# Leonhard111/M3L

Measured on AMD Instinct MI355X. Metric: MAE fwd+bwd samples/sec (image+tactile), higher is better.
Workload: dtype bf16; 1 GPU; BASELINE configs[1]: VTT vision+tactile MAE, 64x64 RGB + 2x32x32 tactile, ViT-Tiny 192/12/3/768 + decoder 192/4/3/768, mask 0.75; batch_per_gpu=256, global_batch=256, parallelism=dp1, grad_allreduce=none (one rank), rccl_ranks=0, step=zero_grad + mask + fwd + bwd + grad all-reduce + Adam

## Files before the change

include/m3l_amd.h:

```cpp
#ifndef M3L_AMD_H
#define M3L_AMD_H
#include <stddef.h>
#include <stdint.h>

#ifdef __cplusplus
extern "C" {
#endif

#define M3L_MAX_TACTILES 8

typedef struct m3l_geom {
    int image_h, image_w, image_patch, image_channels;
    int tactile_h, tactile_w, tactile_patch, tactile_channels;
    int num_tactiles;
    int use_vision;
    int use_tactile;
} m3l_geom;

typedef struct m3l_tf_cfg {
    int dim, depth, heads, mlp_dim;
    int project_out;
    int dtype;
    int dim_head;
} m3l_tf_cfg;

typedef struct m3l_dropout {
    float p;
    uint64_t seed;
} m3l_dropout;

int m3l_version(void);
int m3l_last_error(char* buf, size_t n);
int m3l_set_rowln(int enable);
int m3l_set_attn_block(int mode);
int m3l_set_enc_mega(int mode);
void m3l_set_attn_phase_buffer(void* dev_buf);
int m3l_set_defer_join(int on);
int m3l_set_wgrad_inline(int on);
int m3l_side_join(void* stream);
int m3l_comm_available(void);
int m3l_comm_unique_id(void* out128);
int m3l_comm_init(const void* id128, int rank, int world);
int m3l_comm_world(void);
int m3l_comm_allreduce(float* buf, size_t count, void* after_stream);
int m3l_comm_destroy(void);
int m3l_side_fork(void* after_stream, void** side_out);
int m3l_side_mark_pending(void);
void* m3l_side_stream(void);
int m3l_side_pending(void);
int m3l_set_drop_h(int on);
int m3l_set_t192(int on);
int m3l_set_t192_tt(int tt);
int m3l_set_residual_bf16(int on);
int m3l_set_t192_stagger(int lead_mask, int prio_mask);

int m3l_mask_counts(const m3l_geom* g, double ratio, int* counts_host);
int m3l_mask_sample(const m3l_geom* g, double ratio, int B, const float* const* noise, int64_t* masked, int64_t* unmasked,
                    void* stream);

int m3l_mask_sample_counts(const m3l_geom* g, int nm_img, int nm_tac, int B, const float* const* noise, int64_t* masked,
                           int64_t* unmasked, void* stream);

size_t m3l_embed_ws_bytes(const m3l_geom* g, int D, int dtype, int B, int L);
int m3l_embed_fwd(const m3l_geom* g, int D, int dtype, int B, int L, int cnt_img, const int64_t* idx, const float* image,
                  const float* const* tactiles, const void* const* tensors, void* ws, float* tokens, void* stream);
int m3l_embed_bwd(const m3l_geom* g, int D, int dtype, int B, int L, int cnt_img, const int64_t* idx, const float* image,
                  const float* const* tactiles, const void* const* tensors, void* ws, const float* dtokens, float* const* grads,
                  void* stream);

size_t m3l_transformer_ws_bytes(const m3l_tf_cfg* c, int B, int n);
int m3l_transformer_fwd(const m3l_tf_cfg* c, int B, int n, const float* x_in, const void* const* tensors, void* ws, void* y_t,
                        float* y32, void* stream);
int m3l_transformer_bwd(const m3l_tf_cfg* c, int B, int n, const float* x_in, const void* const* tensors, void* ws, const void* dy,
                        int dy_dtype, float* dx_in, float* const* grads, void* stream);

int m3l_transformer_bwd_range(const m3l_tf_cfg* c, int B, int n, const float* x_in, const void* const* tensors, void* ws,
                              const void* dy, int dy_dtype, float* dx_in, float* const* grads, int layer_hi, int layer_lo, void* stream);

size_t m3l_transformer_ws_bytes_dropout(const m3l_tf_cfg* c, int B, int n, const m3l_dropout* drop);
int m3l_transformer_fwd_dropout(const m3l_tf_cfg* c, int B, int n, const float* x_in, const void* const* tensors, void* ws, void* y_t,
                                float* y32, const m3l_dropout* drop, void* stream);
int m3l_transformer_bwd_dropout(const m3l_tf_cfg* c, int B, int n, const float* x_in, const void* const* tensors, void* ws, const void* dy,
                                int dy_dtype, float* dx_in, float* const* grads, const m3l_dropout* drop, void* stream);
int m3l_transformer_bwd_range_dropout(const m3l_tf_cfg* c, int B, int n, const float* x_in, const void* const* tensors, void* ws,
                                      const void* dy, int dy_dtype, float* dx_in, float* const* grads, int layer_hi, int layer_lo,
                                      const m3l_dropout* drop, void* stream);

// ... 163 lines not shown
```

m3l_amd/_lib.py:

```python
import ctypes as C
import os

_HERE = os.path.dirname(os.path.abspath(__file__))
LIB_PATH = os.environ.get("M3L_LIB_PATH") or os.path.join(_HERE, "lib", "libm3l_amd.so")

c_p = C.c_void_p
c_i = C.c_int
c_sz = C.c_size_t


class Geom(C.Structure):
    _fields_ = [(n, c_i) for n in ("image_h", "image_w", "image_patch", "image_channels", "tactile_h", "tactile_w",
                                   "tactile_patch", "tactile_channels", "num_tactiles", "use_vision", "use_tactile")]


class CnnCfg(C.Structure):
    _fields_ = [(n, c_i) for n in ("in_channels", "height", "width", "dim", "tactile", "dtype")]


class TfCfg(C.Structure):
    _fields_ = [(n, c_i) for n in ("dim", "depth", "heads", "mlp_dim", "project_out", "dtype", "dim_head")]


class MaeCfg(C.Structure):
    _fields_ = [("geom", Geom), ("enc", TfCfg), ("dec", TfCfg), ("masking_ratio", C.c_double), ("early_conv", c_i), ("learned_pos", c_i)]


class Dropout(C.Structure):
    _fields_ = [("p", C.c_float), ("seed", C.c_uint64)]


class CommPlan(C.Structure):
    _fields_ = [("flat", c_p), ("total", C.c_long), ("min_bucket", C.c_long), ("layers_per_chunk", c_i), ("n_stages", c_i),
                ("stage_end", C.POINTER(C.c_long)), ("sent_out", C.POINTER(C.c_long))]


_SIGS = {
    "m3l_version": (c_i, []),
    "m3l_last_error": (c_i, [C.c_char_p, c_sz]),
    "m3l_set_rowln": (c_i, [c_i]),
    "m3l_set_attn_block": (c_i, [c_i]),
    "m3l_set_attn_phase_buffer": (None, [c_p]),
    "m3l_set_enc_mega": (c_i, [c_i]),
    "m3l_set_drop_h": (c_i, [c_i]),
    "m3l_set_direct_conv": (c_i, [c_i]),
    "m3l_set_t192": (c_i, [c_i]),
    "m3l_set_t192_tt": (c_i, [c_i]),
    "m3l_set_t192_stagger": (c_i, [c_i, c_i]),
    "m3l_set_residual_bf16": (c_i, [c_i]),
    "m3l_set_defer_join": (c_i, [c_i]),
    "m3l_set_wgrad_inline": (c_i, [c_i]),
    "m3l_side_join": (c_i, [c_p]),
    "m3l_side_stream": (c_p, []),
    "m3l_side_fork": (c_i, [c_p, C.POINTER(c_p)]),
    "m3l_side_mark_pending": (c_i, []),
    "m3l_comm_available": (c_i, []),
    "m3l_comm_unique_id": (c_i, [c_p]),
    "m3l_comm_init": (c_i, [c_p, c_i, c_i]),
    "m3l_comm_world": (c_i, []),
    "m3l_comm_allreduce": (c_i, [c_p, c_sz, c_p]),
    "m3l_comm_destroy": (c_i, []),
    "m3l_side_pending": (c_i, []),
    "m3l_mask_counts": (c_i, [C.POINTER(Geom), C.c_double, C.POINTER(c_i)]),
    "m3l_mask_sample": (c_i, [C.POINTER(Geom), C.c_double, c_i, c_p, c_p, c_p, c_p]),
    "m3l_mask_sample_counts": (c_i, [C.POINTER(Geom), c_i, c_i, c_i, c_p, c_p, c_p, c_p]),
    "m3l_embed_ws_bytes": (c_sz, [C.POINTER(Geom), c_i, c_i, c_i, c_i]),
    "m3l_embed_fwd": (c_i, [C.POINTER(Geom), c_i, c_i, c_i, c_i, c_i, c_p, c_p, c_p, c_p, c_p, c_p, c_p]),
    "m3l_embed_bwd": (c_i, [C.POINTER(Geom), c_i, c_i, c_i, c_i, c_i, c_p, c_p, c_p, c_p, c_p, c_p, c_p, c_p]),
    "m3l_transformer_ws_bytes": (c_sz, [C.POINTER(TfCfg), c_i, c_i]),
    "m3l_transformer_fwd": (c_i, [C.POINTER(TfCfg), c_i, c_i, c_p, c_p, c_p, c_p, c_p, c_p]),
    "m3l_transformer_bwd": (c_i, [C.POINTER(TfCfg), c_i, c_i, c_p, c_p, c_p, c_p, c_i, c_p, c_p, c_p]),
    "m3l_transformer_bwd_range": (c_i, [C.POINTER(TfCfg), c_i, c_i, c_p, c_p, c_p, c_p, c_i, c_p, c_p, c_i, c_i, c_p]),
    "m3l_transformer_ws_bytes_dropout": (c_sz, [C.POINTER(TfCfg), c_i, c_i, C.POINTER(Dropout)]),
    "m3l_transformer_fwd_dropout": (c_i, [C.POINTER(TfCfg), c_i, c_i, c_p, c_p, c_p, c_p, c_p, C.POINTER(Dropout), c_p]),
    "m3l_transformer_bwd_dropout": (c_i, [C.POINTER(TfCfg), c_i, c_i, c_p, c_p, c_p, c_p, c_i, c_p, c_p, C.POINTER(Dropout), c_p]),
    "m3l_transformer_bwd_range_dropout": (c_i, [C.POINTER(TfCfg), c_i, c_i, c_p, c_p, c_p, c_p, c_i, c_p, c_p, c_i, c_i, C.POINTER(Dropout), c_p]),
    "m3l_frozen_vit_ws_bytes": (c_sz, [C.POINTER(TfCfg), c_i, c_i]),
    "m3l_frozen_vit_fwd": (c_i, [C.POINTER(TfCfg), C.c_float, c_i, c_i, c_p, c_p, c_p, c_p, c_p]),
    "m3l_unshuffle_ws_bytes": (c_sz, [C.POINTER(Geom), c_i, c_i, c_i, c_i, c_i, c_i]),
    "m3l_unshuffle_fwd": (c_i, [C.POINTER(Geom), c_i, c_i, c_i, c_i, c_i, c_i, c_p, c_p, c_p, c_p, c_p, c_p, c_p, c_p]),
    "m3l_unshuffle_bwd": (c_i, [C.POINTER(Geom), c_i, c_i, c_i, c_i, c_i, c_i, c_p, c_p, c_p, c_p, c_p, c_p, c_p,
# ... 128 lines not shown
```

m3l_amd/csrc/t192.hip:

```cpp
#include <hip/hip_runtime.h>
#include <stdlib.h>
#include <string.h>

#include <algorithm>

#include "common.cuh"
#include "kernels.h"

namespace {


#ifndef T192_ABL
#define T192_ABL 0
#endif
#ifndef T192_NS_TALL
#define T192_NS_TALL 4
#endif
template <int D, int TT, int CP> struct TileCfg {
    static constexpr int KS = D / 32, ND = D / 16;
    static constexpr int BLK = 64 * D;
    static constexpr int CHUNK = 2 * BLK;
    static constexpr int PCB = D / 16, PC = 2 * PCB;
    static constexpr bool HALF = D == 192 && TT == 6 && CP == 1;
    static constexpr int DW = (D == 384 || HALF) ? 2 : 4;
// ... 23 lines not shown
    return v;
}
__device__ __forceinline__ float col4_sum(float v) {
    v = xor16_sum(v);
    v = xor32_sum(v);
    return v;
}

__device__ __forceinline__ int f1_swz(int row) { return ((row >> 1) & 1) | (((row >> 3) & 3) << 1); }
__device__ __forceinline__ Frag<bf16> frag_f1p(const char* blk, int t, int ks, int li, int g) {
    const int row = 8 * (li >> 2) + 4 * t + (li & 3);
    Frag<bf16> f;
    f.v = *reinterpret_cast<const bf16x8*>(blk + (ks >> 1) * 4096 + row * 128 + ((((ks & 1) * 4 + g) ^ f1_swz(row)) << 4));
    return f;
}
__device__ __forceinline__ int f2_swz(int row) { return (4 - (row >> 2)) & 3; }
__device__ __forceinline__ Frag<bf16> frag_f2(const char* blk, int dt, int li, int g) {
    const int row = 16 * dt + li;
    Frag<bf16> f;
    f.v = *reinterpret_cast<const bf16x8*>(blk + row * 64 + ((g ^ f2_swz(row)) << 4));
    return f;
}

__device__ __forceinline__ void dma_f1_piece(const bf16* W, int ldw, int r0, int p, char* dst, int lane) {
    const int kt = p >> 2, rg = p & 3;
    const int row = 8 * rg + (lane >> 3), csrc = (lane & 7) ^ f1_swz(row);
    __builtin_amdgcn_global_load_lds((gl_vp)(W + (long)(r0 + row) * ldw + kt * 64 + csrc * 8), (lds_vp)(dst + kt * 4096 + rg * 1024), 16, 0, 0);
}
__device__ __forceinline__ void dma_f2_piece(const bf16* W, int ldw, int c0, int p, char* dst, int lane) {
    const int row = 16 * p + (lane >> 2), csrc = (lane & 3) ^ f2_swz(row);
    __builtin_amdgcn_global_load_lds((gl_vp)(W + (long)row * ldw + c0 + csrc * 8), (lds_vp)(dst + p * 1024), 16, 0, 0);
}

template <int D, int TT, int CP, int LK = 0, typename Issue>
__device__ __forceinline__ void dma_ring(int dw, int nc, char* ring, Issue issue, int tail) {
    using Cf = TileCfg<D, TT, CP>;
    constexpr int LOOK = LK > 0 ? LK : Cf::NSTAGE - 1;
    const int nst = (nc + CP - 1) / CP;
    auto stage = [&](int s) {
        char* dst = ring + (s % Cf::NSTAGE) * Cf::STAGE;
#pragma unroll
        for (int j = 0; j < Cf::PPW; ++j) {
            const int p = dw * Cf::PPW + j, q = p / Cf::PC;
            issue(min(s * CP + q, nc - 1), dst + q * Cf::CHUNK, p % Cf::PC);
        }
    };
    for (int s = 0; s < LOOK && s < nst; ++s) stage(s);
    for (int s = 0; s < nst; ++s) {
        const int ahead = min(LOOK - 1, nst - 1 - s);
        if (ahead >= 4) wait_vmcnt<(LOOK >= 5 ? 4 : 0) * Cf::PPW>();
        else if (ahead == 3) wait_vmcnt<(LOOK >= 4 ? 3 : 0) * Cf::PPW>();
        else if (ahead == 2) wait_vmcnt<(LOOK >= 3 ? 2 : 0) * Cf::PPW>();
        else if (ahead == 1) wait_vmcnt<Cf::PPW>();
        else wait_vmcnt<0>();
        __builtin_amdgcn_s_barrier();
        if (s + LOOK < nst) stage(s + LOOK);
    }
    for (int i = 0; i < tail; ++i) __builtin_amdgcn_s_barrier();
}

template <int KS>
__device__ __forceinline__ void load_tok_frags(const bf16* __restrict__ X, long lrow, bool ok, int g, Frag<bf16> (&fb)[KS]) {
    constexpr int D = 32 * KS;
    uint4 v[KS];
#pragma unroll
    for (int ks = 0; ks < KS; ++ks) v[ks] = *reinterpret_cast<const uint4*>(X + lrow * D + ks * 32 + 8 * g);
#pragma unroll
    for (int ks = 0; ks < KS; ++ks) fb[ks].v = __builtin_bit_cast(bf16x8, ok ? v[ks] : uint4{0u, 0u, 0u, 0u});
}
__device__ __forceinline__ __amdgpu_buffer_rsrc_t rows_rsrc(const void* p, long bytes) {
    return __builtin_amdgcn_make_buffer_rsrc(const_cast<void*>(p), 0, p ? (int)bytes : 0, 0x00020000);
}
constexpr int ROW_OOB = 0x7fffffff;
__device__ __forceinline__ void store_row16(__amdgpu_buffer_rsrc_t r, int rowoff, int byteoff, f32x4 v) {
    __builtin_amdgcn_raw_buffer_store_b128(__builtin_bit_cast(u4v_t, v), r, (int)((unsigned)rowoff + (unsigned)byteoff), 0, 0);
}
__device__ __forceinline__ void store_row8(__amdgpu_buffer_rsrc_t r, int rowoff, int byteoff, bf16x4 v) {
    __builtin_amdgcn_raw_buffer_store_b64(__builtin_bit_cast(u2v_t, v), r, (int)((unsigned)rowoff + (unsigned)byteoff), 0, 0);
}

template <typename R> __device__ __forceinline__ void store_res4(__amdgpu_buffer_rsrc_t r, int rowoff, int col, f32x4 v) {
    if (sizeof(R) == 4) store_row16(r, rowoff, col * 4, v);
    else store_row8(r, rowoff, col * 2, pack_bf16x4(v));
}

template <int TT, int CP, int ND>
// ... 194 lines not shown
        }
#pragma unroll
        for (int st2 = KS; st2 < 2 * KS; ++st2) {
            const Frag<bf16> a0 = fr[st2 % PFD][0], a1 = fr[st2 % PFD][1];
            asm volatile("" ::: "memory");
            if (st2 + PFD < 2 * KS) req(st2 + PFD, fr[st2 % PFD]);
            asm volatile("" ::: "memory");
            if (!(T192_ABL & 4)) {
            yacc[2 * (st2 - KS)] = mma16(a0, hb, yacc[2 * (st2 - KS)]);
            yacc[2 * (st2 - KS) + 1] = mma16(a1, hb, yacc[2 * (st2 - KS) + 1]);
            } else { yacc[2 * (st2 - KS)][0] += (float)hb.v[st2 & 7]; }
        }
    }
    reduce_to_parity0<TT, CP, ND>(RING, tw, cp, lane, yacc);
    if (cp == 0 && (!(T192_ABL & 8) || yacc[0][0] == 1234.5f)) {
        f32x4 r1[ND];
#pragma unroll
        for (int d = 0; d < ND; ++d) r1[d] = ld_res4<R>(x1 + lrow * D + 16 * d + 4 * g);
        asm volatile("" ::: "memory");
        const __amdgpu_buffer_rsrc_t rxo = rows_rsrc(xout, (long)M * D * sizeof(R));
#pragma unroll
        for (int d = 0; d < ND; ++d) {
            const int col = 16 * d + 4 * g;
            const f32x4 v = yacc[d] + *reinterpret_cast<const f32x4*>(B2 + col) + r1[d];
            store_res4<R>(rxo, xoff, col, v);
        }
    }
}

template <int D, int TT, int CP> struct MlpBwdLayout {
    static constexpr bool CS_LDS = D == 192 && !TileCfg<D, TT, CP>::HALF && (CP > 1 || T192_NS_TALL <= 4);
    static constexpr int RING = 0, CS = TileCfg<D, TT, CP>::RING;
    static size_t total(int mlp) { return (size_t)CS + (CS_LDS ? (size_t)TT * mlp * 4 : 0) + D * 4; }
};

template <int ND, typename R>
__device__ __forceinline__ void ln_bwd_rows(const f32x4 (&yacc)[ND], const R* __restrict__ x, const float* G,
                                            const R* __restrict__ dres, R* __restrict__ dx_out, bf16* __restrict__ dxt_out, float eps,
                                            long trow, long lrow, long M, bool active, char* lp_base, int wave, int lane) {
    constexpr int T_D = 16 * ND;
    const int g = lane >> 4, li = lane & 15;
    constexpr int BT = ND % 6 == 0 ? 6 : 4;
    static_assert(ND % BT == 0, "ND is a multiple of the batch");
    const bool use = active && !(T192_ABL & 32);
    const R* xr = x + lrow * T_D + 4 * g;
    float s = 0.f;
#pragma unroll
    for (int d0 = 0; d0 < ND; d0 += BT) {
        f32x4 v[BT];
#pragma unroll
        for (int j = 0; j < BT; ++j) v[j] = ld_res4<R>(xr + 16 * (d0 + j));
#pragma unroll
        for (int j = 0; j < BT; ++j) {
            if (!use) v[j] = f32x4{0.f, 0.f, 0.f, (float)(d0 + j)};
            s += (v[j][0] + v[j][1]) + (v[j][2] + v[j][3]);
        }
    }
    const float mean = col4_sum(s) * (1.0f / T_D);
    asm volatile("" : "+v"(xr));
    float q = 0.f, s1 = 0.f, t2 = 0.f;
#pragma unroll
    for (int d0 = 0; d0 < ND; d0 += BT) {
        f32x4 v[BT];
#pragma unroll
        for (int j = 0; j < BT; ++j) v[j] = ld_res4<R>(xr + 16 * (d0 + j));
#pragma unroll
        for (int j = 0; j < BT; ++j) {
            const int d = d0 + j;
            if (!use) v[j] = f32x4{0.f, 0.f, 0.f, (float)d};
            const f32x4 xc = v[j] - mean;
            q += (xc[0] * xc[0] + xc[1] * xc[1]) + (xc[2] * xc[2] + xc[3] * xc[3]);
            const f32x4 gd = yacc[d] * *reinterpret_cast<const f32x4*>(G + 16 * d + 4 * g);
            s1 += (gd[0] + gd[1]) + (gd[2] + gd[3]);
            const f32x4 t = gd * xc;
            t2 += (t[0] + t[1]) + (t[2] + t[3]);
        }
    }
    const float rstd = rsqrtf(col4_sum(q) * (1.0f / T_D) + eps);
    s1 = col4_sum(s1) * (1.0f / T_D);
    const float s2 = col4_sum(t2) * rstd * (1.0f / T_D);
    asm volatile("" : "+v"(xr));
    __builtin_amdgcn_s_barrier();
    float* LP = reinterpret_cast<float*>(lp_base) + wave * 3 * T_D;
    const int roff32 = use ? (int)(trow * T_D * sizeof(R)) : ROW_OOB, roff16 = use ? (int)(trow * T_D * 2) : ROW_OOB;
    const __amdgpu_buffer_rsrc_t rdx = rows_rsrc(dx_out, M * T_D * sizeof(R)), rdt = rows_rsrc(dxt_out, M * T_D * 2);
    constexpr int BO = 4;
    static_assert(ND % BO == 0, "ND is a multiple of the batch");
    const R* dr_ = dres + lrow * T_D + 4 * g;
#pragma unroll
    for (int d0 = 0; d0 < ND; d0 += BO) {
        f32x4 v[BO], dr[BO];
#pragma unroll
        for (int j = 0; j < BO; ++j) {
            v[j] = ld_res4<R>(xr + 16 * (d0 + j));
            dr[j] = ld_res4<R>(dr_ + 16 * (d0 + j));
        }
        asm volatile("" ::: "memory");
#pragma unroll
        for (int j = 0; j < BO; ++j) {
            const int d = d0 + j, col = 16 * d + 4 * g;
            if (!use) v[j] = f32x4{0.f, 0.f, 0.f, (float)d};
            const f32x4 xh = (v[j] - mean) * rstd;
            const f32x4 gd = yacc[d] * *reinterpret_cast<const f32x4*>(G + col);
            f32x4 rr = f32x4{0.f, 0.f, 0.f, 0.f};
            if (active) rr = (gd - s1 - xh * s2) * rstd;
            if (use) rr += dr[j];
            store_res4<R>(rdx, roff32, col, rr);
            bf16x4 pk;
            pk[0] = (bf16)rr[0]; pk[1] = (bf16)rr[1]; pk[2] = (bf16)rr[2]; pk[3] = (bf16)rr[3];
            store_row8(rdt, roff16, col * 2, pk);
            f32x4 pg = yacc[d] * xh, pb = yacc[d], pc = rr;
            if (!active) { pg = f32x4{0.f, 0.f, 0.f, 0.f}; pb = pg; }
#pragma unroll
            for (int e = 0; e < 4; ++e) {
                pg[e] = row16_sum_t(pg[e]); pb[e] = row16_sum_t(pb[e]); pc[e] = row16_sum_t(pc[e]);
            }
            if (li == 0) {
                *reinterpret_cast<f32x4*>(LP + col) = pg;
                *reinterpret_cast<f32x4*>(LP + T_D + col) = pb;
                *reinterpret_cast<f32x4*>(LP + 2 * T_D + col) = pc;
            }
        }
    }
    asm volatile("s_waitcnt lgkmcnt(0)" ::: "memory");
    __builtin_amdgcn_s_barrier();
}

template <int D, int TT, int CP, typename R>
__global__ __launch_bounds__((TileCfg<D, TT, CP>::THREADS), (TileCfg<D, TT, CP>::MINW)) void mlp_t192_bwd_kernel(const bf16* __restrict__ dxt, R* __restrict__ dx,
                                                                   const R* __restrict__ x1, const float* __restrict__ ln2_w,
                                                                   const bf16* __restrict__ u, const bf16* __restrict__ W2T,
                                                                   const bf16* __restrict__ W1T, float eps, int M, int mlp,
                                                                   bf16* __restrict__ du_out, bf16* __restrict__ dx1t_out,
                                                                   float* __restrict__ cs_part, float* __restrict__ ln_part) {
    using Cf = TileCfg<D, TT, CP>;
    using Lay = MlpBwdLayout<D, TT, CP>;
    constexpr int NCW = Cf::NCW, KS = Cf::KS, ND = Cf::ND;
    static_assert(Lay::CS_LDS || CP == 1, "global column-sum rows are per (tile, wave)");
    extern __shared__ __attribute__((aligned(16))) char smem[];
    char* RING = smem + Lay::RING;
    float* CS = reinterpret_cast<float*>(smem + Lay::CS);
    float* G = Lay::CS_LDS ? CS + TT * mlp : CS;
    const int tid = threadIdx.x, lane = tid & 63, wave = __builtin_amdgcn_readfirstlane(tid >> 6);
    const int g = lane >> 4, li = lane & 15;
    const long row0 = (long)blockIdx.x * Cf::ROWS;
    const int NC = mlp >> 5;
    const int NS = (NC + CP - 1) / CP;

    if (wave >= NCW) {
        dma_ring<D, TT, CP>(wave - NCW, NC, RING, [&](int c, char* dst, int p) {
            if (p < Cf::PCB) dma_f1_piece(W2T, D, 32 * c, p, dst, lane);
            else dma_f2_piece(W1T, mlp, 32 * c, p - Cf::PCB, dst + Cf::BLK, lane);
        }, CP > 1 ? 5 : 3);
        return;
    }
    const int tw = wave % TT, cp = wave / TT;
    const long trow = row0 + 16 * tw + li;
    const bool ok = trow < M;
    Frag<bf16> db[KS];
    load_tok_frags(dxt, ok ? trow : (long)M - 1, ok, g, db);
    for (int id = tid; id < D; id += 64 * NCW) G[id] = ln2_w[id];
    float* CSw = Lay::CS_LDS ? CS + tw * mlp : cs_part + ((long)blockIdx.x * TT + tw) * mlp;

    f32x4 yacc[ND];
#pragma unroll
    for (int d = 0; d < ND; ++d) yacc[d] = f32x4{0.f, 0.f, 0.f, 0.f};
    uint4 un = uint4{0u, 0u, 0u, 0u};
    if (ok && cp < NC) un = *reinterpret_cast<const uint4*>(u + trow * mlp + 32 * cp + 8 * g);

    for (int st = 0; st < NS; ++st) {
        __builtin_amdgcn_s_barrier();
        asm volatile("" ::: "memory");
        const int c = st * CP + cp;
        if (c >= NC) continue;
        const Frag<bf16> uc = {__builtin_bit_cast(bf16x8, un)};
        if (ok && c + CP < NC && !(T192_ABL & 128)) un = *reinterpret_cast<const uint4*>(u + trow * mlp + 32 * (c + CP) + 8 * g);
        const char* Wa = RING + (st % Cf::NSTAGE) * Cf::STAGE + cp * Cf::CHUNK;
        const char* Wb = Wa + Cf::BLK;
        f32x4 ta[2] = {f32x4{0.f, 0.f, 0.f, 0.f}, f32x4{0.f, 0.f, 0.f, 0.f}};
        Frag<bf16> fr[PFD][2];
        auto req = [&](int step, Frag<bf16>(&dst)[2]) {
            if (step < KS) {
                dst[0] = frag_f1p(Wa, 0, step, li, g);
                dst[1] = frag_f1p(Wa, 1, step, li, g);
            } else {
                dst[0] = frag_f2(Wb, 2 * (step - KS), li, g);
                dst[1] = frag_f2(Wb, 2 * (step - KS) + 1, li, g);
            }
        };
#pragma unroll
        for (int i = 0; i < PFD; ++i) req(i, fr[i]);
#pragma unroll
        for (int ks = 0; ks < KS; ++ks) {
            const Frag<bf16> a0 = fr[ks % PFD][0], a1 = fr[ks % PFD][1];
            asm volatile("" ::: "memory");
            req(ks + PFD, fr[ks % PFD]);
            asm volatile("" ::: "memory");
            ta[0] = mma16(a0, db[ks], ta[0]);
            ta[1] = mma16(a1, db[ks], ta[1]);
        }
        Frag<bf16> dub;
#pragma unroll
        for (int j = 0; j < 8; ++j) {
            const float t = j < 4 ? ta[0][j & 3] : ta[1][j & 3];
            dub.v[j] = (bf16)(t * gelu_grad_fast((float)uc.v[j]));
        }
        if (ok && !(T192_ABL & 64)) *reinterpret_cast<bf16x8*>(du_out + trow * mlp + 32 * c + 8 * g) = dub.v;
        {
            float cs[8];
#pragma unroll
            for (int j = 0; j < 8; ++j) cs[j] = row16_sum_t(ok ? (float)dub.v[j] : 0.f);
            if (li == 0) {
                *reinterpret_cast<f32x4*>(CSw + 32 * c + 8 * g) = f32x4{cs[0], cs[1], cs[2], cs[3]};
                *reinterpret_cast<f32x4*>(CSw + 32 * c + 8 * g + 4) = f32x4{cs[4], cs[5], cs[6], cs[7]};
            }
        }
#pragma unroll
        for (int st2 = KS; st2 < 2 * KS; ++st2) {
            const Frag<bf16> a0 = fr[st2 % PFD][0], a1 = fr[st2 % PFD][1];
            asm volatile("" ::: "memory");
            if (st2 + PFD < 2 * KS) req(st2 + PFD, fr[st2 % PFD]);
            asm volatile("" ::: "memory");
            yacc[2 * (st2 - KS)] = mma16(a0, dub, yacc[2 * (st2 - KS)]);
            yacc[2 * (st2 - KS) + 1] = mma16(a1, dub, yacc[2 * (st2 - KS) + 1]);
        }
    }
    reduce_to_parity0<TT, CP, ND>(RING, tw, cp, lane, yacc);
    {
        const R* dres = dx;
        if (sizeof(R) == 2) dres = reinterpret_cast<const R*>(dxt);
        ln_bwd_rows<ND, R>(yacc, x1, G, dres, sizeof(R) == 2 ? nullptr : dx, dx1t_out, eps, trow, ok ? trow : (long)M - 1, M, ok && cp == 0, RING, wave, lane);
    }
    {
        const float* LP0 = reinterpret_cast<const float*>(RING);
        for (int id = tid; id < 3 * D; id += 64 * NCW) {
            float a = 0.f;
#pragma unroll
            for (int w = 0; w < TT; ++w) a += LP0[w * 3 * D + id];
            ln_part[(long)blockIdx.x * 3 * D + id] = a;
        }
        if (Lay::CS_LDS) {
            for (int id = tid; id < mlp; id += 64 * NCW) {
                float a = 0.f;
#pragma unroll
                for (int w = 0; w < TT; ++w) a += CS[w * mlp + id];
                cs_part[(long)blockIdx.x * mlp + id] = a;
            }
        }
    }
    __builtin_amdgcn_s_barrier();
}

template <int D, int TT, int CP>
__global__ __launch_bounds__((TileCfg<D, TT, CP>::THREADS), (TileCfg<D, TT, CP>::MINW)) void mlp_t192_bwd_stg_kernel(const bf16* __restrict__ dxt, float* __restrict__ dx,
                                                                   const float* __restrict__ x1, const float* __restrict__ ln2_w,
                                                                   const bf16* __restrict__ u, const bf16* __restrict__ W2T,
                                                                   const bf16* __restrict__ W1T, float eps, int M, int mlp,
                                                                   bf16* __restrict__ du_out, bf16* __restrict__ dx1t_out,
                                                                   float* __restrict__ cs_part, float* __restrict__ ln_part, int lead_mask, int prio_mask) {
    using Cf = TileCfg<D, TT, CP>;
// ... 694 lines not shown
    if (!(t192_state() > 0 && dtype == 1 && width_ok(D) && mlp % 32 == 0 && mlp >= 32 && M > 0 && rows_fit_32bit(D, M))) return 0;
    if (D == 192) return mlp <= 1024;
    return mlp <= 2048 && (M >= wide_min_rows(D) || forced());
}

static int t192_min_tiles() {
    static const int v = getenv("M3L_T192_MIN_TILES") ? atoi(getenv("M3L_T192_MIN_TILES")) : 128;
    return v;
}
static int g_tall_tt = 0;
static int tall_tt() {
    if (!g_tall_tt) g_tall_tt = (getenv("M3L_T192_TT") && atoi(getenv("M3L_T192_TT")) == 6) ? 6 : 12;
    return g_tall_tt;
}
extern "C" int m3l_set_t192_tt(int tt) {
    const int old = tall_tt();
    g_tall_tt = tt == 6 ? 6 : 12;
    return old;
}
static int g_stg = -1, g_prio = 0;
static void stg_init() {
    if (g_stg < 0) {
        g_stg = getenv("M3L_T192_STG") ? (int)strtol(getenv("M3L_T192_STG"), nullptr, 0) : 0;
        g_prio = getenv("M3L_T192_PRIO") ? (int)strtol(getenv("M3L_T192_PRIO"), nullptr, 0) : 0;
    }
}
extern "C" int m3l_set_t192_stagger(int lead_mask, int prio_mask) {
    stg_init();
    const int old = g_stg;
    g_stg = lead_mask & 0x1fff;
    g_prio = prio_mask & 0xfff;
    return old;
}
static int t192_tt(int M) { return (cdiv(M, 192) >= t192_min_tiles() || forced()) ? tall_tt() : 3; }
static int tile_rows(int D, int M) { return D == 192 ? 16 * t192_tt(M) : 16 * (D == 256 ? WideTile<256>::TT : WideTile<384>::TT); }
int m3l_mlp_t192_tiles(int D, int M) { return cdiv(M, tile_rows(D, M)); }
int m3l_mlp_t192_cs_rows(int D, int M) {
    const int tt = tile_rows(D, M) / 16;
    const bool cs_lds = D == 192 && tt != 6 && (tt == 3 || T192_NS_TALL <= 4);
    return m3l_mlp_t192_tiles(D, M) * (cs_lds ? 1 : tt);
}

template <typename K> static int lds_attr(K kern, size_t bytes) {
    M3L_HIP(hipFuncSetAttribute((const void*)kern, hipFuncAttributeMaxDynamicSharedMemorySize, (int)std::min(bytes, (size_t)160 * 1024)));
    return 0;
}
#define LDS_ONCE(KERN, BYTES)                               \
    {                                                       \
        static int once = -1;                               \
        if (once < 0) once = lds_attr(KERN, BYTES);         \
        if (once) return once;                              \
    }
#define T192_DISPATCH(DV, TTV, ...)                                                                    \
    if ((DV) == 192 && (TTV) == 12) { constexpr int D = 192, TT = 12, CP = 1; __VA_ARGS__; }           \
    else if ((DV) == 192 && (TTV) == 6) { constexpr int D = 192, TT = 6, CP = 1; __VA_ARGS__; }        \
    else if ((DV) == 192) { constexpr int D = 192, TT = 3, CP = 2; __VA_ARGS__; }                      \
    else if ((DV) == 256) { constexpr int D = 256, TT = WideTile<256>::TT, CP = 1; __VA_ARGS__; }      \
    else { constexpr int D = 384, TT = WideTile<384>::TT, CP = 1; __VA_ARGS__; }
#define T192_DISPATCH_FULL(DV, ...)                                                                    \
    if ((DV) == 192 && tall_tt() == 12) { constexpr int D = 192, TT = 12, CP = 1; __VA_ARGS__; }       \
    else if ((DV) == 192) { constexpr int D = 192, TT = 6, CP = 1; __VA_ARGS__; }                      \
    else if ((DV) == 256) { constexpr int D = 256, TT = WideTile<256>::TT, CP = 1; __VA_ARGS__; }      \
    else { constexpr int D = 384, TT = WideTile<384>::TT, CP = 1; __VA_ARGS__; }

#define T192_RES(...)                                            \
    if (m3l_call_rb()) { using R = bf16; __VA_ARGS__; }           \
// ... 27 lines not shown
    const int tt = Dm == 192 ? t192_tt(M) : tile_rows(Dm, M) / 16;
    const double rsz = m3l_call_rb() ? 2.0 : 4.0;
    ProfScope prof("mlp_t192_fwd", M, mlp, tt, 4.0 * M * (double)Dm * mlp, st, (double)M * (Dm * 2.0 + 2.0 * rsz * Dm + mlp * (h ? 4.0 : 2.0)));
    ProArgs none;
    memset(&none, 0, sizeof(none));
    T192_DISPATCH(Dm, tt, T192_RES({
        LDS_ONCE((mlp_t192_fwd_kernel<D, TT, CP, 0, R>), (MlpFwdLayout<D, TT, CP>::total(D == 192 ? 1024 : 2048)));
        mlp_t192_fwd_kernel<D, TT, CP, 0, R><<<cdiv(M, 16 * TT), TileCfg<D, TT, CP>::THREADS, MlpFwdLayout<D, TT, CP>::total(mlp), st>>>(
            (const bf16*)xn2, (const R*)x1, (const bf16*)w1, b1, (const bf16*)w2, b2, M, mlp, (bf16*)u, (bf16*)h, (R*)xout, none);
    }));
    M3L_LAUNCH_CHECK();
    return 0;
}

int m3l_attn_tail_mlp_t192_supported(int dtype, int D, int HD, int mlp, int M, int dim_head) {
    if (!(m3l_mlp_t192_supported(dtype, D, mlp, M) && HD == D && dim_head == 64)) return 0;
    return D != 192 || cdiv(M, 192) >= t192_min_tiles() || forced();
}
int m3l_attn_tail_mlp_t192_fwd(int Dm, int M, int mlp, const void* o, const float* x, const void* wo, const float* bo, const float* ln2_w,
                               const float* ln2_b, float eps, float* x1, void* xn2, const void* w1, const float* b1, const void* w2,
                               const float* b2, void* u, void* h, float* xout, hipStream_t st) {
    M3L_CHECK(width_ok(Dm), "attn_tail_mlp_t192_fwd: width %d", Dm);
    ProfScope prof("attn_tail_mlp_t192_fwd", M, mlp, Dm == 192 ? tall_tt() : tile_rows(Dm, M) / 16, 4.0 * M * (double)Dm * mlp + 2.0 * M * (double)Dm * Dm, st,
                   (double)M * (Dm * 4.0 + 3.0 * (m3l_call_rb() ? 2.0 : 4.0) * Dm + mlp * (h ? 4.0 : 2.0)));
    ProArgs pa = {(const bf16*)o, x, (const bf16*)wo, bo, ln2_w, ln2_b, eps, x1, (bf16*)xn2};
    T192_DISPATCH_FULL(Dm, T192_RES({
        LDS_ONCE((mlp_t192_fwd_kernel<D, TT, CP, 1, R>), (MlpFwdLayout<D, TT, CP>::total(D == 192 ? 1024 : 2048)));
        mlp_t192_fwd_kernel<D, TT, CP, 1, R><<<cdiv(M, 16 * TT), TileCfg<D, TT, CP>::THREADS, MlpFwdLayout<D, TT, CP>::total(mlp), st>>>(
            nullptr, nullptr, (const bf16*)w1, b1, (const bf16*)w2, b2, M, mlp, (bf16*)u, (bf16*)h, (R*)xout, pa);
    }));
    M3L_LAUNCH_CHECK();
    return 0;
}

int m3l_mlp_t192_bwd(int Dm, int M, int mlp, const void* dxt, float* dx, const float* x1, const float* ln2_w, const void* u, const void* w2T,
                     const void* w1T, float eps, void* du, void* dx1t, float* cs_part, float* ln_part, hipStream_t st) {
    M3L_CHECK(width_ok(Dm), "mlp_t192_bwd: width %d", Dm);
    const int tt = Dm == 192 ? t192_tt(M) : tile_rows(Dm, M) / 16;
    ProfScope prof("mlp_t192_bwd", M, mlp, tt, 4.0 * M * (double)Dm * mlp, st,
                   (double)M * (Dm * 4.0 + (m3l_call_rb() ? 2.0 : 12.0) * Dm + mlp * 4.0));
    T192_DISPATCH(Dm, tt, T192_RES({
        LDS_ONCE((mlp_t192_bwd_kernel<D, TT, CP, R>), (MlpBwdLayout<D, TT, CP>::total(D == 192 ? 1024 : 2048)));
        M3L_CHECK((MlpBwdLayout<D, TT, CP>::total(mlp)) <= (size_t)160 * 1024, "mlp_t192_bwd: %zu bytes of LDS", (MlpBwdLayout<D, TT, CP>::total(mlp)));
        stg_init();
        const int stg = g_stg, prio = g_prio;
        if constexpr (D == 192 && TT == 12 && CP == 1 && T192_NS_TALL == 4 && sizeof(R) == 4) {
            if (stg || prio) {
                LDS_ONCE((mlp_t192_bwd_stg_kernel<D, TT, CP>), (MlpBwdLayout<D, TT, CP>::total(1024)));
                mlp_t192_bwd_stg_kernel<D, TT, CP><<<cdiv(M, 16 * TT), TileCfg<D, TT, CP>::THREADS, MlpBwdLayout<D, TT, CP>::total(mlp), st>>>(
                    (const bf16*)dxt, dx, x1, ln2_w, (const bf16*)u, (const bf16*)w2T, (const bf16*)w1T, eps, M, mlp, (bf16*)du, (bf16*)dx1t, cs_part,
                    ln_part, stg & 0xfff, prio);
                M3L_LAUNCH_CHECK();
                return 0;
            }
        }
        mlp_t192_bwd_kernel<D, TT, CP, R><<<cdiv(M, 16 * TT), TileCfg<D, TT, CP>::THREADS, MlpBwdLayout<D, TT, CP>::total(mlp), st>>>(
            (const bf16*)dxt, (R*)dx, (const R*)x1, ln2_w, (const bf16*)u, (const bf16*)w2T, (const bf16*)w1T, eps, M, mlp, (bf16*)du, (bf16*)dx1t, cs_part,
            ln_part);
    }));
    M3L_LAUNCH_CHECK();
    return 0;
}

int m3l_qkv_bwd_t192_supported(int dtype, int D, int K, int M) {
    if (!(t192_state() > 0 && dtype == 1 && width_ok(D) && K % 64 == 0 && K >= 64 && M > 0 && rows_fit_32bit(D, M))) return 0;
    if (D == 192) return cdiv(M, 192) >= t192_min_tiles() || forced();
    return M >= wide_min_rows(D) || forced();
}
int m3l_qkv_bwd_t192_tiles(int D, int M) { return cdiv(M, D == 192 ? 16 * tall_tt() : tile_rows(D, M)); }

int m3l_qkv_bwd_t192(int Dm, int M, int K, const void* dqkv, const float* x, const float* ln1_w, const void* wqkvT, const float* dres, float eps,
                     float* dx_out, void* dxt_out, float* ln_part, hipStream_t st) {
    M3L_CHECK(width_ok(Dm), "qkv_bwd_t192: width %d", Dm);
    ProfScope prof("qkv_bwd_t192", M, K, Dm, 2.0 * M * (double)Dm * K, st,
                   (double)M * (K * 2.0 + Dm * 2.0 + (m3l_call_rb() ? 4.0 : 12.0) * Dm));
    T192_DISPATCH_FULL(Dm, T192_RES({
        LDS_ONCE((qkv_bwd_t192_kernel<D, TT, R>), (QkvBwdLayout<D, TT>::TOTAL));
        qkv_bwd_t192_kernel<D, TT, R><<<cdiv(M, 16 * TT), TileCfg<D, TT, CP>::THREADS, QkvBwdLayout<D, TT>::TOTAL, st>>>(
            (const bf16*)dqkv, (const R*)x, ln1_w, (const bf16*)wqkvT, (const R*)dres, eps, M, K, (R*)dx_out, (bf16*)dxt_out, ln_part);
    }));
    M3L_LAUNCH_CHECK();
    return 0;
}

int m3l_attn_t192_fwd_supported(int dtype, int D, int heads, int n, int B, int dim_head) {
    static const int attn_on = getenv("M3L_T192_ATTN") ? atoi(getenv("M3L_T192_ATTN")) : 1;
    const bool shape = dim_head == 64 && ((D == 192 && heads == 3) || (D == 256 && heads == 4));
    return attn_on > 0 && t192_state() > 0 && dtype == 1 && shape && n > 48 && n <= 192 && (B >= t192_min_tiles() || forced());
// ... 48 lines not shown
```

Measured before the change: 72870 samples/s.

## Offload MLP backward du stores to dedicated store waves via LDS double buffer

In the 192-wide, 12-row-tile MLP backward kernel, two of the DMA waves become store waves. Compute waves write the gelu-grad du chunk into a swizzled, double-buffered LDS area, and the store waves drain it to global memory with buffer stores one stage behind. This takes the scattered global du writes off the compute waves' critical path, at the cost of fewer DMA waves, extra LDS use and extra lgkmcnt waits. Separately, the LN backward helper now keeps bf16 residual rows in registers across its three passes instead of reloading them.

```diff
diff --git a/include/m3l_amd.h b/include/m3l_amd.h
--- a/include/m3l_amd.h
+++ b/include/m3l_amd.h
@@ -53,6 +53,8 @@
 int m3l_set_t192_tt(int tt);
 int m3l_set_residual_bf16(int on);
 int m3l_set_t192_stagger(int lead_mask, int prio_mask);
+int m3l_set_t192_bwd_stores(int mode);
+int m3l_mlp_t192_bwd_store_waves(int D, int M, int mlp);
 
 int m3l_mask_counts(const m3l_geom* g, double ratio, int* counts_host);
 int m3l_mask_sample(const m3l_geom* g, double ratio, int B, const float* const* noise, int64_t* masked, int64_t* unmasked,
diff --git a/m3l_amd/_lib.py b/m3l_amd/_lib.py
--- a/m3l_amd/_lib.py
+++ b/m3l_amd/_lib.py
@@ -47,6 +47,8 @@
     "m3l_set_t192": (c_i, [c_i]),
     "m3l_set_t192_tt": (c_i, [c_i]),
     "m3l_set_t192_stagger": (c_i, [c_i, c_i]),
+    "m3l_set_t192_bwd_stores": (c_i, [c_i]),
+    "m3l_mlp_t192_bwd_store_waves": (c_i, [c_i, c_i, c_i]),
     "m3l_set_residual_bf16": (c_i, [c_i]),
     "m3l_set_defer_join": (c_i, [c_i]),
     "m3l_set_wgrad_inline": (c_i, [c_i]),
diff --git a/m3l_amd/csrc/t192.hip b/m3l_amd/csrc/t192.hip
--- a/m3l_amd/csrc/t192.hip
+++ b/m3l_amd/csrc/t192.hip
@@ -79,26 +79,28 @@
     __builtin_amdgcn_global_load_lds((gl_vp)(W + (long)row * ldw + c0 + csrc * 8), (lds_vp)(dst + p * 1024), 16, 0, 0);
 }
 
-template <int D, int TT, int CP, int LK = 0, typename Issue>
+template <int D, int TT, int CP, int LK = 0, int NDW = 0, typename Issue>
 __device__ __forceinline__ void dma_ring(int dw, int nc, char* ring, Issue issue, int tail) {
     using Cf = TileCfg<D, TT, CP>;
     constexpr int LOOK = LK > 0 ? LK : Cf::NSTAGE - 1;
+    constexpr int PPW = NDW > 0 ? Cf::PC * CP / NDW : Cf::PPW;
+    static_assert(NDW == 0 || ((Cf::PC * CP) % NDW == 0 && (Cf::NSTAGE - 2) * PPW < 64), "whole pieces per DMA wave, vmcnt immediates");
     const int nst = (nc + CP - 1) / CP;
     auto stage = [&](int s) {
         char* dst = ring + (s % Cf::NSTAGE) * Cf::STAGE;
 #pragma unroll
-        for (int j = 0; j < Cf::PPW; ++j) {
-            const int p = dw * Cf::PPW + j, q = p / Cf::PC;
+        for (int j = 0; j < PPW; ++j) {
+            const int p = dw * PPW + j, q = p / Cf::PC;
             issue(min(s * CP + q, nc - 1), dst + q * Cf::CHUNK, p % Cf::PC);
         }
     };
     for (int s = 0; s < LOOK && s < nst; ++s) stage(s);
     for (int s = 0; s < nst; ++s) {
         const int ahead = min(LOOK - 1, nst - 1 - s);
-        if (ahead >= 4) wait_vmcnt<(LOOK >= 5 ? 4 : 0) * Cf::PPW>();
-        else if (ahead == 3) wait_vmcnt<(LOOK >= 4 ? 3 : 0) * Cf::PPW>();
-        else if (ahead == 2) wait_vmcnt<(LOOK >= 3 ? 2 : 0) * Cf::PPW>();
-        else if (ahead == 1) wait_vmcnt<Cf::PPW>();
+        if (ahead >= 4) wait_vmcnt<(LOOK >= 5 ? 4 : 0) * PPW>();
+        else if (ahead == 3) wait_vmcnt<(LOOK >= 4 ? 3 : 0) * PPW>();
+        else if (ahead == 2) wait_vmcnt<(LOOK >= 3 ? 2 : 0) * PPW>();
+        else if (ahead == 1) wait_vmcnt<PPW>();
         else wait_vmcnt<0>();
         __builtin_amdgcn_s_barrier();
         if (s + LOOK < nst) stage(s + LOOK);
@@ -359,7 +361,10 @@
     static constexpr bool CS_LDS = D == 192 && !TileCfg<D, TT, CP>::HALF && (CP > 1 || T192_NS_TALL <= 4);
     static constexpr int RING = 0, CS = TileCfg<D, TT, CP>::RING;
     static size_t total(int mlp) { return (size_t)CS + (CS_LDS ? (size_t)TT * mlp * 4 : 0) + D * 4; }
+    static constexpr int DU_BUF = 16 * TT * 64, DU_BYTES = 2 * DU_BUF;
+    static size_t total_sw(int mlp) { return total(mlp) + DU_BYTES; }
 };
+__device__ __forceinline__ int du_swz(int row) { return (row >> 1) & 3; }
 
 template <int ND, typename R>
 __device__ __forceinline__ void ln_bwd_rows(const f32x4 (&yacc)[ND], const R* __restrict__ x, const float* G,
@@ -367,16 +372,38 @@
                                             long trow, long lrow, long M, bool active, char* lp_base, int wave, int lane) {
     constexpr int T_D = 16 * ND;
     const int g = lane >> 4, li = lane & 15;
+    constexpr bool HOLD = sizeof(R) == 2;
     constexpr int BT = ND % 6 == 0 ? 6 : 4;
     static_assert(ND % BT == 0, "ND is a multiple of the batch");
     const bool use = active && !(T192_ABL & 32);
     const R* xr = x + lrow * T_D + 4 * g;
+    u2v_t xp[HOLD ? ND : 1];
+    if constexpr (HOLD) {
+#pragma unroll
+        for (int d = 0; d < ND; ++d) xp[d] = *reinterpret_cast<const u2v_t*>(xr + 16 * d);
+    }
+    auto x_piece = [&](int d) -> f32x4 {
+        if constexpr (HOLD) {
+            const bf16x4 v = __builtin_bit_cast(bf16x4, xp[d]);
+            return f32x4{(float)v[0], (float)v[1], (float)v[2], (float)v[3]};
+        } else {
+            return ld_res4<R>(xr + 16 * d);
+        }
+    };
+    auto next_pass = [&]() {
+        if constexpr (HOLD) {
+#pragma unroll
+            for (int d = 0; d < ND; ++d) asm volatile("" : "+v"(xp[d]));
+        } else {
+            asm volatile("" : "+v"(xr));
+        }
+    };
     float s = 0.f;
 #pragma unroll
     for (int d0 = 0; d0 < ND; d0 += BT) {
         f32x4 v[BT];
 #pragma unroll
-        for (int j = 0; j < BT; ++j) v[j] = ld_res4<R>(xr + 16 * (d0 + j));
+        for (int j = 0; j < BT; ++j) v[j] = x_piece(d0 + j);
 #pragma unroll
         for (int j = 0; j < BT; ++j) {
             if (!use) v[j] = f32x4{0.f, 0.f, 0.f, (float)(d0 + j)};
@@ -384,13 +411,13 @@
         }
     }
     const float mean = col4_sum(s) * (1.0f / T_D);
-    asm volatile("" : "+v"(xr));
+    next_pass();
     float q = 0.f, s1 = 0.f, t2 = 0.f;
 #pragma unroll
     for (int d0 = 0; d0 < ND; d0 += BT) {
         f32x4 v[BT];
 #pragma unroll
-        for (int j = 0; j < BT; ++j) v[j] = ld_res4<R>(xr + 16 * (d0 + j));
+        for (int j = 0; j < BT; ++j) v[j] = x_piece(d0 + j);
 #pragma unroll
         for (int j = 0; j < BT; ++j) {
             const int d = d0 + j;
@@ -406,7 +433,7 @@
     const float rstd = rsqrtf(col4_sum(q) * (1.0f / T_D) + eps);
     s1 = col4_sum(s1) * (1.0f / T_D);
     const float s2 = col4_sum(t2) * rstd * (1.0f / T_D);
-    asm volatile("" : "+v"(xr));
+    next_pass();
     __builtin_amdgcn_s_barrier();
     float* LP = reinterpret_cast<float*>(lp_base) + wave * 3 * T_D;
     const int roff32 = use ? (int)(trow * T_D * sizeof(R)) : ROW_OOB, roff16 = use ? (int)(trow * T_D * 2) : ROW_OOB;
@@ -419,7 +446,7 @@
         f32x4 v[BO], dr[BO];
 #pragma unroll
         for (int j = 0; j < BO; ++j) {
-            v[j] = ld_res4<R>(xr + 16 * (d0 + j));
+            v[j] = x_piece(d0 + j);
             dr[j] = ld_res4<R>(dr_ + 16 * (d0 + j));
         }
         asm volatile("" ::: "memory");
@@ -453,7 +480,7 @@
     __builtin_amdgcn_s_barrier();
 }
 
-template <int D, int TT, int CP, typename R>
+template <int D, int TT, int CP, typename R, int SW = 0>
 __global__ __launch_bounds__((TileCfg<D, TT, CP>::THREADS), (TileCfg<D, TT, CP>::MINW)) void mlp_t192_bwd_kernel(const bf16* __restrict__ dxt, R* __restrict__ dx,
                                                                    const R* __restrict__ x1, const float* __restrict__ ln2_w,
                                                                    const bf16* __restrict__ u, const bf16* __restrict__ W2T,
@@ -464,18 +491,53 @@
     using Lay = MlpBwdLayout<D, TT, CP>;
     constexpr int NCW = Cf::NCW, KS = Cf::KS, ND = Cf::ND;
     static_assert(Lay::CS_LDS || CP == 1, "global column-sum rows are per (tile, wave)");
+    static_assert(SW == 0 || (D == 192 && TT == 12 && CP == 1 && Lay::CS_LDS && SW < Cf::DW && TT % SW == 0), "store waves: the <192, 12, 1> tile");
+    constexpr int NDMA = Cf::DW - SW;
     extern __shared__ __attribute__((aligned(16))) char smem[];
     char* RING = smem + Lay::RING;
     float* CS = reinterpret_cast<float*>(smem + Lay::CS);
     float* G = Lay::CS_LDS ? CS + TT * mlp : CS;
+    char* DU = reinterpret_cast<char*>(G + D);
     const int tid = threadIdx.x, lane = tid & 63, wave = __builtin_amdgcn_readfirstlane(tid >> 6);
     const int g = lane >> 4, li = lane & 15;
     const long row0 = (long)blockIdx.x * Cf::ROWS;
     const int NC = mlp >> 5;
     const int NS = (NC + CP - 1) / CP;
 
+    if (SW > 0 && wave >= NCW + NDMA) {
+        constexpr int PP = TT / (SW > 0 ? SW : 1);
+        const int sw = wave - NCW - NDMA;
+        const __amdgpu_buffer_rsrc_t rdu = rows_rsrc(du_out, (long)M * mlp * 2);
+        unsigned roff[PP];
+#pragma unroll
+        for (int j = 0; j < PP; ++j) {
+            const int row = 16 * (sw * PP + j) + (lane >> 2);
+            roff[j] = (unsigned)((row0 + row) * mlp * 2) + (unsigned)(16 * ((lane & 3) ^ du_swz(row)));
+        }
+        auto drain = [&](int c) {
+            const char* src = DU + (c & 1) * Lay::DU_BUF + sw * PP * 1024 + lane * 16;
+            u4v_t v[PP];
+#pragma unroll
+            for (int j = 0; j < PP; ++j) v[j] = *reinterpret_cast<const u4v_t*>(src + j * 1024);
+            asm volatile("s_waitcnt lgkmcnt(0)" ::: "memory");
+            if (T192_ABL & 64) return;
+#pragma unroll
+            for (int j = 0; j < PP; ++j) __builtin_amdgcn_raw_buffer_store_b128(v[j], rdu, (int)(roff[j] + (unsigned)(64 * c)), 0, 0);
+        };
+        for (int st = 0; st < NS; ++st) {
+            __builtin_amdgcn_s_barrier();
+            asm volatile("" ::: "memory");
+            if (st > 0) drain(st - 1);
+        }
+        __builtin_amdgcn_s_barrier();
+        asm volatile("" ::: "memory");
+        drain(NS - 1);
+        __builtin_amdgcn_s_barrier();
+        __builtin_amdgcn_s_barrier();
+        return;
+    }
     if (wave >= NCW) {
-        dma_ring<D, TT, CP>(wave - NCW, NC, RING, [&](int c, char* dst, int p) {
+        dma_ring<D, TT, CP, 0, NDMA>(wave - NCW, NC, RING, [&](int c, char* dst, int p) {
             if (p < Cf::PCB) dma_f1_piece(W2T, D, 32 * c, p, dst, lane);
             else dma_f2_piece(W1T, mlp, 32 * c, p - Cf::PCB, dst + Cf::BLK, lane);
         }, CP > 1 ? 5 : 3);
@@ -494,8 +556,10 @@
     for (int d = 0; d < ND; ++d) yacc[d] = f32x4{0.f, 0.f, 0.f, 0.f};
     uint4 un = uint4{0u, 0u, 0u, 0u};
     if (ok && cp < NC) un = *reinterpret_cast<const uint4*>(u + trow * mlp + 32 * cp + 8 * g);
+    char* duw = DU + (16 * tw + li) * 64 + ((g ^ du_swz(li)) << 4);
 
     for (int st = 0; st < NS; ++st) {
+        if (SW > 0) asm volatile("s_waitcnt lgkmcnt(0)" ::: "memory");
         __builtin_amdgcn_s_barrier();
         asm volatile("" ::: "memory");
         const int c = st * CP + cp;
@@ -532,7 +596,8 @@
             const float t = j < 4 ? ta[0][j & 3] : ta[1][j & 3];
             dub.v[j] = (bf16)(t * gelu_grad_fast((float)uc.v[j]));
         }
-        if (ok && !(T192_ABL & 64)) *reinterpret_cast<bf16x8*>(du_out + trow * mlp + 32 * c + 8 * g) = dub.v;
+        if (SW > 0) *reinterpret_cast<bf16x8*>(duw + (c & 1) * Lay::DU_BUF) = dub.v;
+        else if (ok && !(T192_ABL & 64)) *reinterpret_cast<bf16x8*>(du_out + trow * mlp + 32 * c + 8 * g) = dub.v;
         {
             float cs[8];
 #pragma unroll
@@ -553,6 +618,7 @@
         }
     }
     reduce_to_parity0<TT, CP, ND>(RING, tw, cp, lane, yacc);
+    if (SW > 0) asm volatile("s_waitcnt lgkmcnt(0)" ::: "memory");
     {
         const R* dres = dx;
         if (sizeof(R) == 2) dres = reinterpret_cast<const R*>(dxt);
@@ -1313,6 +1379,26 @@
     g_prio = prio_mask & 0xfff;
     return old;
 }
+constexpr int T192_BWD_NSW = 2;
+static int g_bwd_stores = -1;
+static int bwd_stores() {
+    if (g_bwd_stores < 0) {
+        const int v = getenv("M3L_T192_BWD_STORES") ? atoi(getenv("M3L_T192_BWD_STORES")) : 1;
+        g_bwd_stores = v > 0;
+    }
+    return g_bwd_stores;
+}
+extern "C" int m3l_set_t192_bwd_stores(int mode) {
+    const int old = bwd_stores();
+    g_bwd_stores = mode > 0;
+    return old;
+}
+static int t192_tt(int M);
+extern "C" int m3l_mlp_t192_bwd_store_waves(int D, int M, int mlp) {
+    if (D != 192 || T192_NS_TALL != 4 || t192_tt(M) != 12) return 0;
+    const bool fits = MlpBwdLayout<192, 12, 1>::total_sw(mlp) <= (size_t)160 * 1024 && ((long)M + 256) * mlp * 2 < 2147483647L;
+    return fits && bwd_stores() ? T192_BWD_NSW : 0;
+}
 static int t192_tt(int M) { return (cdiv(M, 192) >= t192_min_tiles() || forced()) ? tall_tt() : 3; }
 static int tile_rows(int D, int M) { return D == 192 ? 16 * t192_tt(M) : 16 * (D == 256 ? WideTile<256>::TT : WideTile<384>::TT); }
 int m3l_mlp_t192_tiles(int D, int M) { return cdiv(M, tile_rows(D, M)); }
@@ -1406,6 +1492,16 @@
     M3L_LAUNCH_CHECK();
     return 0;
 }
+
+#define T192_BWD_SW(SWv)                                                                                                                      \
+    {                                                                                                                                         \
+        LDS_ONCE((mlp_t192_bwd_kernel<D, TT, CP, R, SWv>), (size_t)160 * 1024);                                                               \
+        mlp_t192_bwd_kernel<D, TT, CP, R, SWv><<<cdiv(M, 16 * TT), TileCfg<D, TT, CP>::THREADS, lds_sw, st>>>(                                \
+            (const bf16*)dxt, (R*)dx, (const R*)x1, ln2_w, (const bf16*)u, (const bf16*)w2T, (const bf16*)w1T, eps, M, mlp, (bf16*)du,        \
+            (bf16*)dx1t, cs_part, ln_part);                                                                                                   \
+        M3L_LAUNCH_CHECK();                                                                                                                   \
+        return 0;                                                                                                                             \
+    }
 
 int m3l_mlp_t192_bwd(int Dm, int M, int mlp, const void* dxt, float* dx, const float* x1, const float* ln2_w, const void* u, const void* w2T,
                      const void* w1T, float eps, void* du, void* dx1t, float* cs_part, float* ln_part, hipStream_t st) {
@@ -1428,6 +1524,11 @@
                 return 0;
             }
         }
+        if constexpr (D == 192 && TT == 12 && CP == 1 && T192_NS_TALL == 4) {
+            const size_t lds_sw = MlpBwdLayout<D, TT, CP>::total_sw(mlp);
+            const int sw = m3l_mlp_t192_bwd_store_waves(Dm, M, mlp);
+            if (sw > 0) T192_BWD_SW(T192_BWD_NSW)
+        }
         mlp_t192_bwd_kernel<D, TT, CP, R><<<cdiv(M, 16 * TT), TileCfg<D, TT, CP>::THREADS, MlpBwdLayout<D, TT, CP>::total(mlp), st>>>(
             (const bf16*)dxt, (R*)dx, (const R*)x1, ln2_w, (const bf16*)u, (const bf16*)w2T, (const bf16*)w1T, eps, M, mlp, (bf16*)du, (bf16*)dx1t, cs_part,
             ln_part);
```

Result: no change. 73670 samples/s (median of 6 runs) (+1.1%).
